# TuringLang/AdvancedVI.jl

Measured on AMD Instinct MI355X. Metric: ELBO-grad-estimates/sec, higher is better.
Workload: dtype f32

## Files before the change

### advancedvi.jl_amd/csrc/api_batch.hip

```cpp
#include "api_common.h"

bool graph_capturable(const mivi_ctx *c) {
  return c->target == TGT_DIAG_GAUSS || c->target == TGT_DENSE_GAUSS || c->target == TGT_FUNNEL || c->target == TGT_LOGREG;
}
mivi_status_t reserve_target(mivi_ctx *c, int M) {
  if (c->target == TGT_LOGREG && !logreg_reserve(c, M)) return fail(c, MIVI_ERR_HIP, "logistic regression: scratch allocation failed");
  return MIVI_OK;
}

static mivi_status_t record_chain(mivi_ctx *k, const void *params, uint64_t first, uint64_t stride, int cnt, const uint64_t *idx_ptr, void *value,
                                  void *grad) {
  Chain chn;
  chn.on = true;
  chn.estimates_only = true;
  mivi_status_t s = MIVI_OK;
  for (int i = 0; i < cnt && s == MIVI_OK; ++i) {
    RngArgs r = rng_of(k, first + (uint64_t)i * stride);
    if (idx_ptr) r.idx_ptr = idx_ptr;
    k->cur = i & 1;
    chn.has_next = (i + 1 < cnt);
    chn.next_rng = rng_of(k, first + ((uint64_t)i + 1) * stride);
    chn.next_rng.idx_ptr = r.idx_ptr;
    s = run_estimate(k, params, r, k->cfg.n_mc, 1, final_out(k, value, grad), &chn);
  }
// ... 205 lines not shown
    fs.stl = stl ? 1 : 0;
    if (st == steps - 1 && (value_last || grad_last)) { fs.lane_last = Llast - 1; fs.grad_last = grad_last; fs.value_last = value_last; }
    if (dist) { fs.parts = (char *)t.parts.p + (size_t)(overlap ? (st & 1) : 0) * (size_t)t.cap_LP * part_len * 4; fs.part_stride = (long long)part_len; }
    return fs;
  };
  ExchangePipe &pipe = c->fb_pipe;
  int handed = 0;
  auto step = [&](int st) -> mivi_status_t {
    const FbStep fs = make_step(st);
    if (overlap && (s = pipe.reuse(c, c->stream, st))) return s;
    fb_launch_eps(c, fs, st == 0, c->stream);
    fb_launch_compute(c, fs, c->stream);
    if (!dist) return MIVI_OK;
    hipStream_t xs = c->stream;
    if (overlap) {
      if ((s = pipe.hand_over(c, c->stream, st, &xs))) return s;
      handed = st + 1;
    }
    if ((s = dist_allreduce_f32(c, fs.parts, (size_t)fs.L * part_len, xs))) return s;
    fb_launch_finalize_parts(c, fs, xs);
    return overlap ? pipe.finish(c, st) : MIVI_OK;
  };
  s = MIVI_OK;
  for (int st = 0; st < steps && s == MIVI_OK; ++st) s = step(st);
  if (s) {
    pipe.join_after_error(c->stream, handed);
    return s;
  }
  if (overlap && (s = pipe.join(c, c->stream, steps))) return s;
  HIPCHK(c, hipGetLastError());
  return MIVI_OK;
}

mivi_status_t mivi::fb_objective(mivi_ctx *c, const void *params, uint64_t idx, int lanes, int entropy, void *values) {
  if (!fb_route(c, params, nullptr, nullptr) || c->M_total != c->cfg.n_mc) return MIVI_ERR_UNSUPPORTED;
  return fb_batch(c, params, idx, lanes, nullptr, nullptr, values, nullptr, entropy);
}

int32_t mivi_batch_lanes(const mivi_ctx_t *c, int32_t count) {
  if (!c || count <= 0) return 0;
  const int Lmax = switches().fb_lanes, steps = (count + Lmax - 1) / Lmax;
  return (count + steps - 1) / steps;
}

int32_t mivi_batch_info(const mivi_ctx_t *c, const void *params, int32_t what) {
  if (!c) return 0;
  if (what == 1) return 3;
  if (what == 2) return 4;
  if (what == 3) return c->exchange_lost ? 1 : 0;
  if (what == 4) return c->graph_records;
  if (what == 5) return live_allocations();
  if (what == 6) return live_handles();
  if (what == 7) return c->last_loop;
  return (what == 0 && params && fb_route(c, params, nullptr, nullptr)) ? 1 : 0;
}

mivi_status_t mivi_profile_batch(mivi_ctx_t *c, const void *params, int32_t lanes, int32_t reps, double *us_out) {
  if (!c || !params || lanes <= 0 || reps <= 0 || !us_out) return MIVI_ERR_BAD_ARG;
  if (mivi_status_t rs = refuse_non_gaussian(c, "mivi_profile_batch")) return rs;
  (void)hipSetDevice(c->cfg.device);
  if (!fb_route(c, params, nullptr, nullptr)) return fail(c, MIVI_ERR_UNSUPPORTED, "mivi_profile_batch: this configuration does not take the batch engine");
  if (lanes > switches().fb_lanes) lanes = switches().fb_lanes;
  char *o = (char *)c->tmp_out.p;
  mivi_status_t s = fb_batch(c, params, 1, lanes, o, o + 16, nullptr, nullptr);
  if (s) return s;
  const FbTab *tab = fb_prepare(c, c->cfg.n_mc, lanes);
  if (!tab) return fail(c, MIVI_ERR_HIP, "batch engine: work table allocation failed");
  FbStep fs{};
  fs.params = params; fs.M = c->cfg.n_mc; fs.L = lanes; fs.tab = tab;
  fs.rng = rng_of(c, 1);
  fs.grads = c->fb.grads.p; fs.grad_stride = (long long)mivi_params_len(c); fs.values = c->fb.values.p; fs.value_stride = 1; fs.lane_last = -1;
  fs.dense = c->target == TGT_DENSE_GAUSS ? 1 : 0;
  fs.stl = stl_entropy(c) ? 1 : 0;
  us_out[3] = us_out[4] = 0.0;
  EventTimer timer;
  for (int which = 0; which < 5; ++which) {
    if ((which == 3 && !fs.dense) || (which == 4 && !fs.stl)) continue;
    for (int r = -2; r < reps; ++r) {
      if (r == 0 && (s = timer.start(c, c->stream))) return s;
      if (which == 0) fb_launch_eps(c, fs, true, c->stream);
      else fb_launch_compute(c, fs, c->stream, which == 1 ? 1 : (which == 2 ? 2 : (which == 3 ? 4 : 8)));
    }
    double us = 0.0;
    if ((s = timer.stop_us(c, c->stream, &us))) return s;
    us_out[which] = us / reps;
  }
  HIPCHK(c, hipGetLastError());
  return MIVI_OK;
}

bool fb_dist_route(const mivi_ctx *c, const void *params, const void *grad) { return fb_route(c, params, grad, nullptr) && fb_whole_tiles(c, c->cfg.n_mc); }
mivi_status_t fb_batch_dist(mivi_ctx *c, const void *params, uint64_t idx0, int count, void *value, void *grad) {
  return fb_batch(c, params, idx0, count, value, grad, nullptr, nullptr, -1, true);
}

mivi_status_t mivi_estimate_gradient_each(mivi_ctx_t *c, const void *params, uint64_t idx0, int32_t count, void *values, void *grads) {
  if (!c || !params || !values || count <= 0) return MIVI_ERR_BAD_ARG;
  (void)hipSetDevice(c->cfg.device);
  if (c->target == TGT_NONE) return fail(c, MIVI_ERR_NO_TARGET, "no target set");
  if (fb_route(c, params, nullptr, grads)) return fb_batch(c, params, idx0, count, nullptr, nullptr, values, grads);
  const size_t plen = (size_t)mivi_params_len(c);
  mivi_status_t s = MIVI_OK;
  for (int i = 0; i < count && s == MIVI_OK; ++i)
    s = run_estimate(c, params, rng_of(c, idx0 + (uint64_t)i), c->cfg.n_mc, 1,
                     final_out(c, (char *)values + (size_t)i * c->esize, grads ? (void *)((char *)grads + (size_t)i * plen * c->esize) : c->tmp_out.p));
  return s;
// ... 128 lines not shown
```

### advancedvi.jl_amd/csrc/api_core.hip

```cpp
#include <atomic>
#include <climits>
#include <cstddef>
#include <cstdlib>

#include "api_common.h"

__global__ void k_acc_value_f32(double *acc, const float *v, double w, int first) { acc[0] = (first ? 0.0 : acc[0]) + w * (double)v[0]; }
__global__ void k_acc_value_f64(double *acc, const double *v, double w, int first) { acc[0] = (first ? 0.0 : acc[0]) + w * v[0]; }
__global__ void k_store_value_f32(float *out, const double *acc) { out[0] = (float)acc[0]; }
__global__ __launch_bounds__(256) void k_mean_values_f32(double *acc, const float *v, int n, double w) {
  __shared__ double part[256];
  double s = 0.0;
  for (int i = threadIdx.x; i < n; i += 256) s += (double)v[i];
  part[threadIdx.x] = s;
  __syncthreads();
  if (threadIdx.x == 0) {
    double t = 0.0;
    for (int i = 0; i < 256; ++i) t += part[i];
    acc[0] = w * t;
  }
}
__global__ void k_store_value_f64(double *out, const double *acc) { out[0] = acc[0]; }
__global__ void k_set_u64x2(uint64_t *dst, uint64_t a, uint64_t b, int n) { dst[0] = a; if (n > 1) dst[1] = b; }
__global__ void k_bump_u64(uint64_t *dst, uint64_t by) { dst[0] += by; }
__global__ void k_empty(int *sink) {
  extern __shared__ int lds_dyn[];
  if (sink && threadIdx.x == 0 && blockIdx.x == 0x7fffffff) sink[0] = lds_dyn[0];
}


mivi_status_t fail(mivi_ctx *c, mivi_status_t s, const char *msg) {
  if (c) c->err = msg;
  return s;
}

namespace mivi {
namespace {
enum SwitchKind {
  SW_PRESENCE,
  SW_ON_UNLESS_0,
  SW_OFF_UNLESS_1,
  SW_INT,
  SW_STRING
};
constexpr int kNoLo = INT_MIN, kNoHi = INT_MAX;
struct SwitchRow { const char *name; SwitchKind kind; size_t field; int def, lo, hi; const char *meaning; };
#define SW(f) offsetof(Switches, f)
const SwitchRow kSwitchTable[] = {
    {"MIVI_FR_GEN1", SW_PRESENCE, SW(fr_gen1), 0, 0, 0, "full-rank f32: first-generation tile kernels at every shape (lds_path_shape_ok)"},
    {"MIVI_STEIN_GEN1", SW_PRESENCE, SW(stein_gen1), 0, 0, 0, "Stein accumulation stage on the first-generation kernel (lds_stein_ok)"},
    {"MIVI_STL_GEN1", SW_PRESENCE, SW(stl_gen1), 0, 0, 0, "sticking-the-landing solve: not the second-generation packed solve (stl2_shape_ok)"},
    {"MIVI_STL_VALU", SW_PRESENCE, SW(stl_valu), 0, 0, 0, "first-generation solve on the vector ALU, not the 16-column look-ahead solve (launch_fr_stl)"},
    {"MIVI_LR_F32_LOGITS", SW_PRESENCE, SW(lr_f32_logits), 0, 0, 0, "logistic regression: f32-MFMA logits kernel (the one d % 4 != 0 takes), no operand planes"},
    {"MIVI_LR_NO_PLANES", SW_PRESENCE, SW(lr_no_planes), 0, 0, 0, "logistic regression: logits with X split in the tile (k_lr_logits_f16x2)"},
    {"MIVI_LR_NO_XPLANES", SW_PRESENCE, SW(lr_no_xplanes), 0, 0, 0, "logistic regression: X^T R with the splits made in the tile (k_lr_xtr_f16x2)"},
    {"MIVI_NO_FUSED_LOOP", SW_PRESENCE, SW(no_fused_loop), 0, 0, 0, "no launch-free loop kernels: batches and optimisation loops as graphs of launches"},
    {"MIVI_NO_FUSED_UPDATE", SW_PRESENCE, SW(no_fused_update), 0, 0, 0, "graph loop: the optimiser step as a kernel of its own, not in the VJP epilogue"},
    {"MIVI_FORCE_EXCHANGE_LOST", SW_PRESENCE, SW(force_exchange_lost), 0, 0, 0, "test hook (tests/test_gpu_loop_oracle.py): the first exchanging loop call counts as lost"},
    {"MIVI_BATCH_GEN3", SW_ON_UNLESS_0, SW(batch_gen3), 0, 0, 0, "=0: batches off the third-generation engine, on the lane-batched second-generation kernels"},
    {"MIVI_FB_STL", SW_ON_UNLESS_0, SW(fb_stl), 0, 0, 0, "=0: sticking-the-landing batches off the engine (lane-batched kernels + solves)"},
    {"MIVI_PROD_QUAD", SW_ON_UNLESS_0, SW(prod_quad), 0, 0, 0, "=0: four lanes' sampling products as k_fr_prod32m tiles, not k_fr_prod32q"},
    {"MIVI_P2P_DIRECT", SW_OFF_UNLESS_1, SW(p2p_direct), 0, 0, 0, "=1: sharded partials staged straight into the peers' buffers (mivi_p2p_partials_direct)"},
    {"MIVI_GRAPH_MIN", SW_INT, SW(graph_min), 6, kNoLo, kNoHi, "smallest full-rank batch that is captured as a graph (shorter: an eager chain)"},
    {"MIVI_CHAINS", SW_INT, SW(chains), 0, kNoLo, kNoHi, "> 0: that many interleaved contexts per batch (0: by shape)"},
    {"MIVI_FB_LANES", SW_INT, SW(fb_lanes), 80, 1, 256, "estimates per step of the batch engine"},
    {"MIVI_LANE_BATCH", SW_INT, SW(lane_batch), -1, kNoLo, kNoHi, "contexts per graph branch: 0 = every context on a branch of its own, 1 .. 4, < 0 = by shape"},
    {"MIVI_VJP_STRIP", SW_INT, SW(vjp_strip), 3, 0, 32, "tiles per workgroup of the lane-batched VJP (k_fr_vjp32s); 0 = one each (k_fr_vjp32m)"},
    {"MIVI_VJP_TILE", SW_INT, SW(vjp_tile), 0, kNoLo, kNoHi, "32 / 64 pins the second-generation VJP's tile size (0: by shape)"},
    {"MIVI_RCCL_LIB", SW_STRING, SW(rccl_lib), 0, 0, 0, "path of the RCCL library to load (unset: the loader's search)"},
#ifdef MIVI_DEV
    {"MIVI_FB_DBG", SW_PRESENCE, SW(fb_dbg), 0, 0, 0, "batch engine: per-workgroup clock stamps, summarised on stderr"},
    {"MIVI_STL_STAMPS", SW_PRESENCE, SW(stl_stamps), 0, 0, 0, "second-generation solve: per-block clock stamps on stderr"},
    {"MIVI_FB_KNOCK", SW_INT, SW(fb_knock), 0, kNoLo, kNoHi, "batch engine: work-skipping bits (operand loads / MFMAs / epilogue / stores)"},
    {"MIVI_FB_RING", SW_INT, SW(fb_ring), 0, kNoLo, kNoHi, "4 / 8 pins the engine product's ring depth (tools/fb_lane_curve.py)"},
    {"MIVI_KNOCK", SW_INT, SW(knock), 0, kNoLo, kNoHi, "second-generation kernels: work-skipping bits"},
#endif
};
#undef SW
Switches read_switches() {
  Switches s{};
  for (const SwitchRow &r : kSwitchTable) {
    const char *v = getenv(r.name);
    void *f = (char *)&s + r.field;
    switch (r.kind) {
      case SW_PRESENCE: *(bool *)f = v != nullptr; break;
      case SW_ON_UNLESS_0: *(bool *)f = !(v && atoi(v) == 0); break;
      case SW_OFF_UNLESS_1: *(bool *)f = v && atoi(v) == 1; break;
      case SW_INT: { const int x = v ? atoi(v) : r.def; *(int *)f = x < r.lo ? r.lo : (x > r.hi ? r.hi : x); break; }
      case SW_STRING: *(const char **)f = v; break;
    }
  }
  return s;
}
}
const Switches &switches() {
  static const Switches s = read_switches();
  return s;
}

bool grid_resident(const mivi_ctx *c, const void *kernel, int block, size_t dyn_lds, long long grid) {
  int nb = 0;
  if (hipOccupancyMaxActiveBlocksPerMultiprocessor(&nb, kernel, block, dyn_lds) != hipSuccess) { (void)hipGetLastError(); return false; }
  return c->n_cu > 0 && (long long)nb * c->n_cu >= grid;
}
}

static std::atomic<int32_t> g_live_allocations{0};
int32_t live_allocations() { return g_live_allocations.load(); }

void mivi::DevBuf::release() {
  if (owned && p) { (void)hipFree(p); --g_live_allocations; }
  p = nullptr; bytes = 0; owned = false;
}

mivi_status_t ensure(mivi_ctx *c, DevBuf &b, size_t bytes, bool zero, bool fine_grained) {
  if (b.bytes >= bytes && b.p) return MIVI_OK;
  b.release();
  if (bytes == 0) bytes = 16;
  void *p = nullptr;
  HIPCHK(c, fine_grained ? hipExtMallocWithFlags(&p, bytes, hipDeviceMallocFinegrained) : hipMalloc(&p, bytes));
  ++g_live_allocations;
  b.p = p; b.bytes = bytes; b.owned = true;
  if (zero) HIPCHK(c, hipMemsetAsync(b.p, 0, bytes, c->stream));
  return MIVI_OK;
}

mivi_status_t ensure_zeroed(mivi_ctx *c, DevBuf &b, size_t bytes) {
// ... 527 lines not shown
```

### advancedvi.jl_amd/csrc/fr_planes.h

```cpp
#pragma once
#include "device_common.h"

namespace mivi {

typedef float f32x16 __attribute__((ext_vector_type(16)));
typedef float f32x4 __attribute__((ext_vector_type(4)));
typedef _Float16 f16x8 __attribute__((ext_vector_type(8)));
typedef _Float16 f16x2 __attribute__((ext_vector_type(2)));
typedef unsigned u32x4v __attribute__((ext_vector_type(4)));

constexpr int kFrag = 512;
constexpr int kSplitProducts = 3;
constexpr float kEpsScale = 2048.f;
constexpr float kEpsInv = 1.f / 2048.f;

#define FB_GLDS16(gptr, lptr, off)                                                                         \
  __builtin_amdgcn_global_load_lds((const __attribute__((address_space(1))) void *)(gptr),                 \
                                   (__attribute__((address_space(3))) void *)(lptr), 16, off, 0)

template <int N>
__device__ __forceinline__ void fb_wait_vm() {
  __builtin_amdgcn_s_waitcnt((N & 15) | (7 << 4) | (15 << 8) | ((N >> 4) << 14));
  asm volatile("" ::: "memory");
}
// ... 30 lines not shown
  return (float)hh[odd] + (float)ll[odd];
}
__device__ __forceinline__ void fb_store_frag(unsigned *dst, const float *x) {
  u32x4v uh, ul;
  fb_split2(x, uh, ul);
  store16_wt(dst, uh);
  store16_wt(dst + 256, ul);
}

constexpr int kStageW = 16 * 256;

template <int WJ>
struct FbFrags {
  u32x4v A[2][2], B[WJ][2];
};
__device__ __forceinline__ f32x16 fb_mma(const u32x4v &a, const u32x4v &b, const f32x16 &c) {
  return __builtin_amdgcn_mfma_f32_32x32x16_f16(__builtin_bit_cast(f16x8, a), __builtin_bit_cast(f16x8, b), c, 0, 0, 0);
}
template <int WJ>
__device__ __forceinline__ void fb_group(const FbFrags<WJ> &F, f32x16 (&acc)[2][WJ]) {
  constexpr int PA[3] = {1, 0, 0}, PB[3] = {0, 1, 0};
#pragma unroll
  for (int p = 0; p < 3; ++p)
#pragma unroll
    for (int i = 0; i < 2; ++i)
#pragma unroll
      for (int j = 0; j < WJ; ++j) acc[i][j] = fb_mma(F.A[i][PA[p]], F.B[j][PB[p]], acc[i][j]);
}

template <int OFF>
__device__ __forceinline__ void fb_group_read_asm(f32x16 &acc0, f32x16 &acc1, const FbFrags<1> &Fc, FbFrags<1> &Fn, unsigned ab, unsigned bb) {
  static_assert(OFF >= 0 && OFF + 3072 < 65536, "ds_read_b128 offset field");
  asm volatile(
      "v_mfma_f32_32x32x16_f16 %[c0], %[a0l], %[bh], %[c0]\n\t"
      "ds_read_b128 %[n0h], %[ab] offset:%[o0]\n\t"
      "ds_read_b128 %[n0l], %[ab] offset:%[o1]\n\t"
      "v_mfma_f32_32x32x16_f16 %[c1], %[a1l], %[bh], %[c1]\n\t"
      "ds_read_b128 %[n1h], %[ab] offset:%[o2]\n\t"
      "ds_read_b128 %[n1l], %[ab] offset:%[o3]\n\t"
      "v_mfma_f32_32x32x16_f16 %[c0], %[a0h], %[bl], %[c0]\n\t"
      "ds_read_b128 %[nbh], %[bb] offset:%[o0]\n\t"
      "v_mfma_f32_32x32x16_f16 %[c1], %[a1h], %[bl], %[c1]\n\t"
      "ds_read_b128 %[nbl], %[bb] offset:%[o1]\n\t"
      "v_mfma_f32_32x32x16_f16 %[c0], %[a0h], %[bh], %[c0]\n\t"
      "v_mfma_f32_32x32x16_f16 %[c1], %[a1h], %[bh], %[c1]\n\t"
      "s_waitcnt lgkmcnt(0)"
      : [c0] "+v"(acc0), [c1] "+v"(acc1), [n0h] "=&v"(Fn.A[0][0]), [n0l] "=&v"(Fn.A[0][1]), [n1h] "=&v"(Fn.A[1][0]), [n1l] "=&v"(Fn.A[1][1]),
        [nbh] "=&v"(Fn.B[0][0]), [nbl] "=&v"(Fn.B[0][1])
      : [a0h] "v"(Fc.A[0][0]), [a0l] "v"(Fc.A[0][1]), [a1h] "v"(Fc.A[1][0]), [a1l] "v"(Fc.A[1][1]), [bh] "v"(Fc.B[0][0]), [bl] "v"(Fc.B[0][1]),
        [ab] "v"(ab), [bb] "v"(bb), [o0] "n"(OFF), [o1] "n"(OFF + 1024), [o2] "n"(OFF + 2048), [o3] "n"(OFF + 3072)
      : "memory");
}

template <int WJ>
__device__ __forceinline__ void fb_read_frags(const unsigned *lds, int slot, int wm, int wn, int lane, FbFrags<WJ> &F) {
  const unsigned *cur = lds + slot * kStageW + 4 * lane;
#pragma unroll
  for (int i = 0; i < 2; ++i)
#pragma unroll
    for (int p = 0; p < 2; ++p) F.A[i][p] = *(const u32x4v *)(cur + ((2 * wm + i) * 2 + p) * 256);
#pragma unroll
  for (int j = 0; j < WJ; ++j)
#pragma unroll
    for (int p = 0; p < 2; ++p) F.B[j][p] = *(const u32x4v *)(cur + (8 + (WJ * wn + j) * 2 + p) * 256);
}

}
```

### advancedvi.jl_amd/csrc/kernels_fullrank_batch.hip

```cpp
#include <algorithm>
#include <cstdlib>
#include <type_traits>
#include <cstdio>
#include <vector>

#include "device_common.h"
#include "fr_elem.h"
#include "fr_planes.h"

#ifndef FB_VK
#define FB_VK 0
#endif
#ifndef FB_WJ
#define FB_WJ 1
#endif

namespace mivi {

struct FbArgs {
  int d, M, L;
  int dT, MT;
  const float *params;
  const float *t_mean, *t_istd;
  unsigned *CA;
// ... 542 lines not shown
#pragma unroll
        for (int g2 = 0; g2 < 2; ++g2) {
          float x[8];
#pragma unroll
          for (int e = 0; e < 8; ++e) x[e] = I[(16 * g2 + 8 * (e >> 2) + 4 * h + (e & 3)) * LDC + l31] * s;
          fb_store_frag(WVl + ((size_t)r32[i] * nmg + 2 * cb32 + g2) * kFrag + 4 * lane, x);
        }
      }
    }
  }
  FB_STAMP(a, 3);
  if (!kDG && !kSU && (flags & 1) && wn == 0 && lane < 32) {
    const int nrb = d >> 5;
#pragma unroll
    for (int i = 0; i < 2; ++i) {
      const int r = 32 * r32[i] + lane;
      float lg, bad;
      logdet_block32(r < a.dT ? a.params[a.dT + (size_t)r * a.dT + r] : 1.f, lg, bad);
      if (lane == 0) {
        a.ld_part[r32[i]] = (double)lg;
        a.ld_part[nrb + r32[i]] = (double)bad;
      }
    }
  }
}

__device__ __forceinline__ void fb_value_block(const FbArgs &a, int l, double *red) {
  const int d = a.d;
  ValueIn vin{};
  vin.ell_const = a.ell_const;
  vin.ell_part = a.ell_part + (size_t)l * a.ell_stride;
  vin.n_ell_part = (d >> 5) * (a.M >> 5);
  vin.he_part = a.he_part + (size_t)l * a.he_stride;
  vin.n_he_part = (d >> 6) * (a.M >> 5);
  vin.ld_part = a.ld_part;
  vin.n_ld_part = d >> 5;
  OutArgs out{};
  const bool last = l == a.lane_last && a.value_last;
  out.value = last ? a.value_last : a.values + (size_t)l * a.value_stride;
  if (a.parts) {
    out.partials_mode = 1;
    out.partials = a.parts + (size_t)l * a.part_stride;
    out.scalars_off = (int64_t)d + (int64_t)(d >> 7) * ((d >> 7) + 1) / 2 * 16384;
  }
  out.ent_kind = a.ent_kind;
  out.M_total = a.M_total;
  out.M_local = a.MT;
  out.status = a.status;
  const float *pp = a.params;
  const int dT = a.dT;
  finalize_value_block<float, 256, false>(dT, vin, out, (int64_t)dT + (int64_t)dT * dT, [pp, dT](int i) { return pp[dT + (size_t)i * dT + i]; }, red);
}

template <int WJ, int NRV, int TABW, int WPE, bool PART = false>
__global__ __launch_bounds__(512 / WJ, WPE / WJ) void k_fb_vjp(FbArgs a) {
  static_assert(WJ == 1, "the transposing B reads are written for the 64 x 32 wave tiles");
  constexpr int LDC = 36, NF = WJ, kPW = 2 * WJ;
  constexpr int NR = NRV;
  constexpr int kBody = (NR * kStageW > 16 * kImgW / 2) ? NR * kStageW : 16 * kImgW / 2;
  __shared__ __attribute__((aligned(16))) unsigned lds[kBody + TABW];
  float *wf = reinterpret_cast<float *>(lds + kBody);
  const int tid = threadIdx.x, lane = tid & 63, l31 = lane & 31, h = lane >> 5;
  const int w = __builtin_amdgcn_readfirstlane(tid >> 6);
  const int wm = w / (4 / WJ), wn = w % (4 / WJ);
  if ((int)blockIdx.x < a.L) {
    if (tid < 256) fb_value_block(a, (int)blockIdx.x, reinterpret_cast<double *>(lds));
    return;
  }
  const __attribute__((address_space(4))) int *wp = (const __attribute__((address_space(4))) int *)a.work + 4 * ((int)blockIdx.x - a.L);
  const int ln = wp[0], rc = wp[1];
  const int rb = rc & 0xffff, cb = rc >> 16;
  const int d = a.d, M = a.M, nmg = M >> 4, dT = a.dT;
  const int row0 = rb * 128, col0 = cb * 128;
  const bool last = ln == a.lane_last && a.grad_last;
  float *grad = last ? a.grad_last : a.grads + (size_t)ln * a.grad_stride;
  const bool upper = a.write_upper || last;
  const int G = nmg;
  const int NB = M >> 7;
  const unsigned *sp[NF];
  unsigned btr;
  {
    const int G4 = lane >> 4, c16 = lane & 15;
    const int kgpar = G4 & 1, hq = G4 >> 1, hp = c16 & 1, half = (c16 >> 1) & 1, sl = 4 * hq + (c16 >> 2);
    btr = 16u * (unsigned)(8 * (2 * hp + kgpar) + ((sl & 7) ^ (4 * hp))) + 8u * (unsigned)half;
  }
#pragma unroll
  for (int f = 0; f < NF; ++f) {
    const int fs = NF * w + f, fr = fs & 3;
    if (fs < 4) {
      sp[f] = a.WV + (size_t)ln * a.plane_stride + ((size_t)((row0 >> 5) + fr) * nmg) * kFrag + 4 * lane;
    } else {
      const int m8 = lane >> 3, s8 = m8 >> 2, hp = (m8 >> 1) & 1, kgpar = m8 & 1, sl = 8 * s8 + ((lane & 7) ^ (4 * hp));
      sp[f] = a.epsP + (size_t)ln * a.plane_stride + ((size_t)((col0 >> 4) + 2 * fr + kgpar)) * kFrag + 4 * (sl + 32 * hp);
    }
  }
  int gi = 0;
  const int bstep_odd = (d >> 4) * kFrag - 64;
  constexpr int kMaxNBv = 16;
  float twi[kMaxNBv];
  auto load_table = [&]() {
    if (tid < 128) {
      const float *wi = a.winv + (size_t)ln * (size_t)NB * d + row0 + tid;
#pragma unroll
      for (int r = 0; r < kMaxNBv; ++r) twi[r] = wi[(size_t)(r < NB ? r : NB - 1) * d];
    }
    asm volatile("" ::: "memory");
  };
  auto build_table = [&]() {
    if (tid < 128) {
// ... 44 lines not shown
  int cj[WJ];
#pragma unroll
  for (int j = 0; j < WJ; ++j) cj[j] = (col0 >> 5) + WJ * wn + j;
  const bool work = cj[0] <= ri[1];
  bool dg[2];
#pragma unroll
  for (int i = 0; i < 2; ++i) {
    dg[i] = false;
#pragma unroll
    for (int j = 0; j < WJ; ++j) dg[i] = dg[i] || ri[i] == cj[j];
  }
  f32x16 acc[2][WJ];
#pragma unroll
  for (int i = 0; i < 2; ++i)
#pragma unroll
    for (int j = 0; j < WJ; ++j)
#pragma unroll
      for (int r = 0; r < 16; ++r) acc[i][j][r] = 0.f;
  double rsd[2] = {0.0, 0.0};
  float rcur[2] = {0.f, 0.f};
  auto after_group = [&](auto S, int g, const FbFrags<WJ> &F) {
    if (__builtin_expect(dg[0] || dg[1], 0)) {
#pragma unroll
      for (int i = 0; i < 2; ++i)
        if (dg[i]) {
#pragma unroll
          for (int e = 0; e < 8; ++e) rcur[i] += fb_unsplit2(F.A[i][0], F.A[i][1], e);
        }
    }
    if constexpr (decltype(S)::value == 3 || decltype(S)::value == -1) {
      if (((g + 1) & 7) == 0 && g + 1 < G) {
        const float *wr = wf + ((g >> 3) << 7) + 64 * wm;
#pragma unroll
        for (int i = 0; i < 2; ++i) {
#pragma unroll
          for (int q = 0; q < 4; ++q) {
            const f32x4 f4 = *(const f32x4 *)(wr + 32 * i + 8 * q + 4 * h);
#pragma unroll
            for (int j = 0; j < WJ; ++j)
#pragma unroll
              for (int c = 0; c < 4; ++c) acc[i][j][4 * q + c] *= f4[c];
          }
          rsd[i] = (rsd[i] + (double)rcur[i]) * (double)wr[32 * i + l31];
          rcur[i] = 0.f;
        }
        asm volatile("" ::: "memory");
      }
    }
  };
  auto compute = [&](auto S, int g, const FbFrags<WJ> &F) {
    if (!(FB_VK & 32)) fb_group<WJ>(F, acc);
    after_group(S, g, F);
  };
  {
    FB_STAMP(a, 0);
    FB_NOTE(a, 4, G);
    load_table();
#pragma unroll
    for (int s0 = 0; s0 < NR - 1; ++s0) issue(s0);
    fb_wait_vm<kPW * (NR - 1)>();
    build_table();
    int slot = 0;
    for (int g = 0; g < G; ++g) {
      if (g == 1) FB_STAMP(a, 1);
      if (g + NR - 2 < G) fb_wait_vm<kPW * (NR - 2)>();
      else if (NR > 3 && g + 1 < G) fb_wait_vm<kPW>();
      else fb_wait_vm<0>();
      fb_barrier();
      if (g + NR - 1 < G) issue(slot == 0 ? NR - 1 : slot - 1);
      if (work) {
        FbFrags<WJ> F;
        read_frags(slot, F);
        compute(std::integral_constant<int, -1>{}, g, F);
      }
      slot = slot == NR - 1 ? 0 : slot + 1;
    }
  }
  fb_barrier();
  FB_STAMP(a, 2);
  if ((FB_VK & 128)) return;
  float *Cs = reinterpret_cast<float *>(lds) + w * kImgW;
  const float *wfin = wf + (NB - 1) * 128 + 64 * wm;
  const double invM = 1.0 / (double)a.M_total;
  const bool pow2M = (a.M_total & (a.M_total - 1)) == 0;
  const float invMe = (float)invM * kEpsInv;
  const double direct = direct_entropy_coeff(a.ent_kind);
  const int i4 = 4 * (lane & 7);
#pragma unroll
  for (int i = 0; i < 2; ++i) {
#pragma unroll
    for (int j = 0; j < WJ; ++j) {
      if (cj[j] > ri[i] || 32 * ri[i] >= dT) continue;
      const bool diag = ri[i] == cj[j];
      const int rbase = 32 * ri[i], cbase = 32 * cj[j];
#pragma unroll
      for (int q = 0; q < 4; ++q) {
        const f32x4 v = {acc[i][j][4 * q], acc[i][j][4 * q + 1], acc[i][j][4 * q + 2], acc[i][j][4 * q + 3]};
        *(f32x4 *)(Cs + l31 * LDC + 8 * q + 4 * h) = v;
      }
      const f32x4 ff = *(const f32x4 *)(wfin + 32 * i + i4);
#pragma unroll
      for (int p = 0; p < 4; ++p) {
        const int n = 8 * p + (lane >> 3);
        const int gi = rbase + i4, gj = cbase + n;
        float cjj = 1.f;
        if (diag && gj >= gi && gj < gi + 4) cjj = a.params[dT + (size_t)gj * dT + gj];
        const f32x4 v = *(const f32x4 *)(Cs + n * LDC + i4) * ff;
// ... 230 lines not shown
  const int d = fb_pad(c->cfg.d), M = fb_pad(s.M), L = s.L;
  FbArgs a = fb_args(c, s.params, s.M);
  a.L = L;
  a.rng = s.rng;
  a.obj = s.obj;
  const int gx = (d / 64) * (M / 32) / 2;
  a.n_riders = with_cplanes ? (4 * (d / 32) + gx - 1) / gx : 0;
  hipLaunchKernelGGL(k_fb_eps, dim3(gx, L + a.n_riders), dim3(512), 0, stream, a);
}
void fb_launch_pplanes(mivi_ctx *c, hipStream_t stream) {
  FbArgs a = fb_args(c, nullptr, c->cfg.n_mc);
  hipLaunchKernelGGL(k_fb_pplanes, dim3(c->cfg.d / 32, 4), dim3(512), 0, stream, a);
}
void fb_launch_tplanes(mivi_ctx *c, hipStream_t stream) {
  FbArgs a = fb_args(c, nullptr, c->cfg.n_mc);
  hipLaunchKernelGGL(k_fb_tplanes, dim3(c->cfg.d / 32, 4), dim3(512), 0, stream, a);
}
void fb_launch_compute(mivi_ctx *c, const FbStep &s, hipStream_t stream, int which) {
  const FbTab &tb = *s.tab;
  FbArgs a = fb_args(c, s.params, s.M);
  a.L = s.L;
  a.grads = (float *)s.grads; a.grad_stride = s.grad_stride;
  a.values = (float *)s.values; a.value_stride = s.value_stride;
  a.grad_last = (float *)s.grad_last; a.value_last = (float *)s.value_last; a.lane_last = s.lane_last;
  a.write_upper = s.write_upper;
  a.parts = (float *)s.parts; a.part_stride = s.part_stride;
  if (s.obj) { a.ent_kind = s.ent_kind; a.M_total = s.M; }
#ifdef MIVI_DEV
  static long long *dbg_buf = nullptr;
  const bool dbg_on = switches().fb_dbg;
  if (dbg_on && !dbg_buf) (void)hipMalloc(&dbg_buf, 2 * 8192 * 8 * sizeof(long long));
  auto dump = [&](const char *name, int n) {
    if (!dbg_on) return;
    (void)hipStreamSynchronize(stream);
    std::vector<long long> h((size_t)n * 8);
    (void)hipMemcpy(h.data(), dbg_buf, h.size() * 8, hipMemcpyDeviceToHost);
    long long t0 = h[0], t3 = 0;
    for (int i = 0; i < n; ++i) { t0 = std::min(t0, h[(size_t)i * 8]); t3 = std::max(t3, h[(size_t)i * 8 + 3]); }
    double pro = 0, loop = 0, epi = 0, pg = 0; long long gs = 0;
    for (int i = 0; i < n; ++i) { const long long *r = &h[(size_t)i * 8]; pro += r[1] - r[0]; loop += r[2] - r[1]; epi += r[3] - r[2]; gs += r[4]; }
    pg = loop / (double)gs;
    fprintf(stderr, "[fbdbg] %s: %d workgroups, span %.2f us | mean prologue %.2f us, main loop %.2f us (%.3f us per group), epilogue %.2f us | last start %.2f us\n", name, n, (t3 - t0) * 0.01, pro / n * 0.01, loop / n * 0.01, pg * 0.01, epi / n * 0.01, 0.0);
    std::vector<long long> st; for (int i = 0; i < n; ++i) st.push_back(h[(size_t)i * 8] - t0);
    std::sort(st.begin(), st.end());
    fprintf(stderr, "[fbdbg]   starts (us): p25 %.2f p50 %.2f p75 %.2f p90 %.2f max %.2f\n", st[n / 4] * 0.01, st[n / 2] * 0.01, st[3 * n / 4] * 0.01, st[9 * n / 10] * 0.01, st[n - 1] * 0.01);
  };
  a.dbg = dbg_on ? dbg_buf : nullptr;
  a.knock = switches().fb_knock;
#endif
  a.work = (const int4 *)tb.prod.p; a.n_work = tb.n_prod;
  const int n_cu = c->n_cu > 0 ? c->n_cu : 256;
  auto own_cu_for = [&](int n, bool equal_tiles) {
#ifdef MIVI_DEV
    if (switches().fb_ring == 4) return false;
    if (switches().fb_ring == 8) return true;
#endif
    const int gmax = fb_pad(c->cfg.d) / 16;
    const int thr10 = gmax <= 32 ? 10 : (gmax <= 64 ? 10 + (gmax - 32) * 7 / 32 : kOwnCuTilesPerCU10 + (gmax - 64 < 64 ? gmax - 64 : 64) * 5 / 64);
    return !equal_tiles && n > n_cu && 10 * (long long)n <= (long long)thr10 * n_cu;
  };
  auto prod = [&](auto MODE, int n) {
    constexpr int md = decltype(MODE)::value;
    if (own_cu_for(n, md == FB_DENSE_G)) hipLaunchKernelGGL((k_fb_prod<kWJ, md, 8>), dim3(n), dim3(512 / kWJ), 0, stream, a);
    else hipLaunchKernelGGL((k_fb_prod<kWJ, md, 4>), dim3(n), dim3(512 / kWJ), 0, stream, a);
  };
  if (s.dense) {
    if (which & 1) prod(std::integral_constant<int, FB_DENSE_R>{}, tb.n_prod);
    a.work = (const int4 *)tb.prod2.p; a.n_work = tb.n_prod2;
    if (which & 4) prod(std::integral_constant<int, FB_DENSE_G>{}, tb.n_prod2);
  } else if (which & 1) {
    prod(std::integral_constant<int, FB_DIAG>{}, tb.n_prod);
#ifdef MIVI_DEV
    dump("k_fb_prod<DIAG>", tb.n_prod);
#endif
  }
  if (s.stl && (which & 8)) {
    a.work = (const int4 *)tb.prod3.p; a.n_work = tb.n_prod;
    prod(std::integral_constant<int, FB_STL_U>{}, tb.n_prod);
  }
  a.work = (const int4 *)tb.vjp.p; a.n_work = tb.n_vjp;
  if (s.values_only) {
    if (which & 2) hipLaunchKernelGGL((k_fb_vjp<kWJ, 3, 256, 6>), dim3(s.L), dim3(512 / kWJ), 0, stream, a);
    return;
  }
  if (which & 2) {
    if (s.parts) {
      if (a.M <= 256) hipLaunchKernelGGL((k_fb_vjp<kWJ, 3, 256, 6, true>), dim3(tb.n_vjp + s.L), dim3(512 / kWJ), 0, stream, a);
      else hipLaunchKernelGGL((k_fb_vjp<kWJ, 3, 2048, 4, true>), dim3(tb.n_vjp + s.L), dim3(512 / kWJ), 0, stream, a);
    }
    else if (a.M <= 256) hipLaunchKernelGGL((k_fb_vjp<kWJ, 3, 256, 6>), dim3(tb.n_vjp + s.L), dim3(512 / kWJ), 0, stream, a);
    else hipLaunchKernelGGL((k_fb_vjp<kWJ, 3, 2048, 4>), dim3(tb.n_vjp + s.L), dim3(512 / kWJ), 0, stream, a);
#ifdef MIVI_DEV
    dump("k_fb_vjp", tb.n_vjp);
#endif
  }
}

void fb_launch_finalize_parts(mivi_ctx *c, const FbStep &s, hipStream_t stream) {
  FbArgs a = fb_args(c, s.params, s.M);
  a.L = s.L;
  a.grads = (float *)s.grads; a.grad_stride = s.grad_stride;
  a.values = (float *)s.values; a.value_stride = s.value_stride;
  a.grad_last = (float *)s.grad_last; a.value_last = (float *)s.value_last; a.lane_last = s.lane_last;
  a.write_upper = s.write_upper;
  a.parts = (float *)s.parts; a.part_stride = s.part_stride;
  hipLaunchKernelGGL(k_fb_finalize_parts, dim3(c->cfg.d + 1, s.L), dim3(256), 0, stream, a);
}

}
```

### advancedvi.jl_amd/csrc/mivi_internal.h

```cpp
#pragma once
#include <hip/hip_runtime.h>
#include <math.h>
#include <stdint.h>

#include <string>
#include <utility>
#include <vector>

#include "../../include/mivi.h"
#include "philox.h"
#include "switches.h"

namespace mivi {

constexpr double kLog2Pi = 1.8378770664093454835606594728112;

struct RngArgs {
  uint64_t seed;
  uint64_t idx_base;
  const uint64_t *idx_ptr;
  int m_offset;
};

enum TargetKind : int {
// ... 395 lines not shown
  std::vector<char> h_Z, h_G, h_ell;

  int cap_M = 0;
  mivi::DevBuf eps[2], epsT[2], ell_part[2], he_part[2], sc_part[2], ld_part[2];
  mivi::DevBuf tabA, tabB, tabD;
  mivi::DevBuf stl_CT, stl_Dinv;
  mivi::DevBuf stl_F;
  bool want_stl_pack = false, stl_pack_done = false;
  mivi::DevBuf stl_X;
  mivi::DevBuf lds_tabV, lds_tabV64, lds_tabS;
  int lds_nV = 0, lds_nV64 = 0, lds_nS = 0, lds_M = -1;
  bool d_idx_valid = false;
  uint64_t d_idx_expect = 0;
  mivi::DevBuf lds_tabSt;
  int lds_nSt = 0, lds_st_d = -1;
  mivi::ValueJob *defer_value = nullptr;
  bool value_deferred = false;
  int he_n[2] = {0, 0};
  int nA = 0, nB = 0, nD = 0, tab_M = -1;
  int cur = 0;
  int mf_nblk = 0;
  mivi::DevBuf Z, W, RT, ell, X;
  mivi::DevBuf row_part, status, d_idx, acc, tmp_params, tmp_out;
  mivi::DevBuf obj_vals;
  mivi::DevBuf stein_A, stein_g;
  mivi::DevBuf sg_S, sg_d;
  int sg_cap = 0;
  mivi::DevBuf ms_work, ms_part;
  mivi::DevBuf bam_host;
  mivi::DevBuf ngd_est, natgrad_host;
  mivi::DevBuf h2_acc;
  mivi::DevBuf lowr_E, lowr_V, lowr_prep, lowr_sx, lowr_part;
  int base = MIVI_BASE_NORMAL;
  double base_nu = 0.0, base_c0 = 0.0, base_H = 0.0;
  mivi::DevBuf bd_U, bd_R;
  mivi::DevBuf lp_dinv, lp_scal, lp_work, lp_host;
  mivi::DevBuf dog_part;
  const uint64_t *idx_src = nullptr;
  mivi::EpsSpec pre;
  long long *dbg = nullptr;
  int dP = 0, MP = 0;

  mivi::GraphCache graph;
  int graph_records = 0;
  mivi::FbTables fb;

  int idx_stride = 1;
  bool is_child = false;
  int n_cu = 0;
  size_t lds_max = 64 * 1024;
  bool exchange_lost = false;
  int last_status_bits = 0;
  int last_loop = 0;
  mivi::DevBuf snap;
  mivi_ctx *kids[kMaxKids] = {};
  int n_kids = 0;
  unsigned long long target_gen = 0, kid_gen = ~0ull;
  bool dist_capture_refused = false;
  bool dist_direct = false;
  bool dist_lane4 = false;
  mivi::LaneRecorder *rec = nullptr;
  int lane_id = 0;
  mivi::DevBuf kid_out[kMaxKids];

  ~mivi_ctx() { (void)mivi_comm_destroy(this); graph.drop(); }
};

#pragma GCC visibility push(hidden)
mivi_status_t ensure(mivi_ctx *c, mivi::DevBuf &b, size_t bytes, bool zero, bool fine_grained = false);
mivi_status_t ensure_zeroed(mivi_ctx *c, mivi::DevBuf &b, size_t bytes);
mivi_status_t upload(mivi_ctx *c, mivi::DevBuf &b, const void *src, size_t bytes);
int32_t live_allocations();
mivi_status_t make_stream(mivi_ctx *c, mivi::Stream &s, bool own_queue);
mivi_status_t make_event(mivi_ctx *c, mivi::Event &e, bool timing);
mivi_status_t ensure_pipe(mivi_ctx *c, mivi::ExchangePipe &p, bool own_queue);
int32_t live_handles();
#pragma GCC visibility pop

template <typename F>
inline auto by_dtype(const mivi_ctx *c, F &&f) { return c->cfg.dtype == MIVI_F32 ? f(float{}) : f(double{}); }

namespace mivi {

struct ValueJob;
void launch_mf_main(mivi_ctx *c, const void *params, const RngArgs &rng, int M, int want_grad, const void *G,
                    const ValueIn &vin, const OutArgs &out, const ValueJob *prev = nullptr);
enum DeviceLoopId : int { LOOP_GRAPH = 0, LOOP_MF_SGD = 1, LOOP_LR_SMALL = 2, LOOP_MF_GEN = 3, LOOP_FR_SMALL = 4, LOOP_FR_ROWS = 5, LOOP_MF_FUNNEL_SGD = 6,
                          LOOP_MANY = 16 };
struct LoopBufs {
  void *value, *grad;
  double *rec, *area;
};
struct ManyRun {
  uint64_t seed, idx0;
  double eta, ell_const;
};
struct ManyLaunch {
  int n_runs;
  const ManyRun *runs;
  int *status;
  const void *t_mean, *t_istd;
  const uint8_t *y;
  const void *X;
  long long x_stride;
};
constexpr int kManyGridY = 65535;
// ... 193 lines not shown
```

Baseline: 352,900.

## Add software-pipelined VJP loop overlapping LDS fragment reads with MFMAs

Adds a pipelined variant of the batch-engine VJP kernel. A hand-scheduled inline-asm group interleaves the MFMAs of the current k-group with the ds_read and transposing ds_read_b64_tr_b16 loads of the next group's fragments, using a four-slot ring and double-buffered fragments. The launch picks this variant when M > 256 or the tile count is at most twice the CU count, and it uses 4 waves per EU instead of 6 for the small-M case. The aim is to hide LDS latency behind matrix work, at the cost of more registers and ring LDS, lower occupancy, and a fragile hand-written asm schedule.

```diff
diff --git a/advancedvi.jl_amd/csrc/api_batch.hip b/advancedvi.jl_amd/csrc/api_batch.hip
--- a/advancedvi.jl_amd/csrc/api_batch.hip
+++ b/advancedvi.jl_amd/csrc/api_batch.hip
@@ -281,6 +281,7 @@
   if (what == 5) return live_allocations();
   if (what == 6) return live_handles();
   if (what == 7) return c->last_loop;
+  if (what == 8) return c->last_vjp_pipelined;
   return (what == 0 && params && fb_route(c, params, nullptr, nullptr)) ? 1 : 0;
 }
 
diff --git a/advancedvi.jl_amd/csrc/api_core.hip b/advancedvi.jl_amd/csrc/api_core.hip
--- a/advancedvi.jl_amd/csrc/api_core.hip
+++ b/advancedvi.jl_amd/csrc/api_core.hip
@@ -72,7 +72,7 @@
     {"MIVI_FB_DBG", SW_PRESENCE, SW(fb_dbg), 0, 0, 0, "batch engine: per-workgroup clock stamps, summarised on stderr"},
     {"MIVI_STL_STAMPS", SW_PRESENCE, SW(stl_stamps), 0, 0, 0, "second-generation solve: per-block clock stamps on stderr"},
     {"MIVI_FB_KNOCK", SW_INT, SW(fb_knock), 0, kNoLo, kNoHi, "batch engine: work-skipping bits (operand loads / MFMAs / epilogue / stores)"},
-    {"MIVI_FB_RING", SW_INT, SW(fb_ring), 0, kNoLo, kNoHi, "4 / 8 pins the engine product's ring depth (tools/fb_lane_curve.py)"},
+    {"MIVI_FB_RING", SW_INT, SW(fb_ring), 0, kNoLo, kNoHi, "units 4 / 8 pin the engine product's ring depth (tools/fb_lane_curve.py), tens 3 / 4 the VJP's plain / pipelined loop (tools/fb_vjp_loops.py)"},
     {"MIVI_KNOCK", SW_INT, SW(knock), 0, kNoLo, kNoHi, "second-generation kernels: work-skipping bits"},
 #endif
 };
diff --git a/advancedvi.jl_amd/csrc/fr_planes.h b/advancedvi.jl_amd/csrc/fr_planes.h
--- a/advancedvi.jl_amd/csrc/fr_planes.h
+++ b/advancedvi.jl_amd/csrc/fr_planes.h
@@ -106,6 +106,36 @@
       : "memory");
 }
 
+template <int OFF>
+__device__ __forceinline__ void fb_group_read_tr_asm(f32x16 &acc0, f32x16 &acc1, const FbFrags<1> &Fc, FbFrags<1> &Fn, unsigned ab, unsigned bt) {
+  static_assert(OFF >= 0 && OFF + 3072 < 65536, "ds_read offset field");
+  uint2 bh0, bh1, bl0, bl1;
+  asm volatile(
+      "v_mfma_f32_32x32x16_f16 %[c0], %[a0l], %[bh], %[c0]\n\t"
+      "ds_read_b128 %[n0h], %[ab] offset:%[o0]\n\t"
+      "ds_read_b128 %[n0l], %[ab] offset:%[o1]\n\t"
+      "v_mfma_f32_32x32x16_f16 %[c1], %[a1l], %[bh], %[c1]\n\t"
+      "ds_read_b128 %[n1h], %[ab] offset:%[o2]\n\t"
+      "ds_read_b128 %[n1l], %[ab] offset:%[o3]\n\t"
+      "v_mfma_f32_32x32x16_f16 %[c0], %[a0h], %[bl], %[c0]\n\t"
+      "ds_read_b64_tr_b16 %[bh0], %[bt] offset:%[o0]\n\t"
+      "ds_read_b64_tr_b16 %[bh1], %[bt] offset:%[t1]\n\t"
+      "v_mfma_f32_32x32x16_f16 %[c1], %[a1h], %[bl], %[c1]\n\t"
+      "ds_read_b64_tr_b16 %[bl0], %[bt] offset:%[o1]\n\t"
+      "ds_read_b64_tr_b16 %[bl1], %[bt] offset:%[t3]\n\t"
+      "v_mfma_f32_32x32x16_f16 %[c0], %[a0h], %[bh], %[c0]\n\t"
+      "v_mfma_f32_32x32x16_f16 %[c1], %[a1h], %[bh], %[c1]\n\t"
+      "s_waitcnt lgkmcnt(0)"
+      : [c0] "+v"(acc0), [c1] "+v"(acc1), [n0h] "=&v"(Fn.A[0][0]), [n0l] "=&v"(Fn.A[0][1]), [n1h] "=&v"(Fn.A[1][0]), [n1l] "=&v"(Fn.A[1][1]),
+        [bh0] "=&v"(bh0), [bh1] "=&v"(bh1), [bl0] "=&v"(bl0), [bl1] "=&v"(bl1)
+      : [a0h] "v"(Fc.A[0][0]), [a0l] "v"(Fc.A[0][1]), [a1h] "v"(Fc.A[1][0]), [a1l] "v"(Fc.A[1][1]), [bh] "v"(Fc.B[0][0]), [bl] "v"(Fc.B[0][1]),
+        [ab] "v"(ab), [bt] "v"(bt), [o0] "n"(OFF), [o1] "n"(OFF + 1024), [o2] "n"(OFF + 2048), [o3] "n"(OFF + 3072), [t1] "n"(OFF + 512),
+        [t3] "n"(OFF + 1536)
+      : "memory");
+  Fn.B[0][0] = u32x4v{bh0.x, bh0.y, bh1.x, bh1.y};
+  Fn.B[0][1] = u32x4v{bl0.x, bl0.y, bl1.x, bl1.y};
+}
+
 template <int WJ>
 __device__ __forceinline__ void fb_read_frags(const unsigned *lds, int slot, int wm, int wn, int lane, FbFrags<WJ> &F) {
   const unsigned *cur = lds + slot * kStageW + 4 * lane;
diff --git a/advancedvi.jl_amd/csrc/kernels_fullrank_batch.hip b/advancedvi.jl_amd/csrc/kernels_fullrank_batch.hip
--- a/advancedvi.jl_amd/csrc/kernels_fullrank_batch.hip
+++ b/advancedvi.jl_amd/csrc/kernels_fullrank_batch.hip
@@ -618,9 +618,10 @@
   finalize_value_block<float, 256, false>(dT, vin, out, (int64_t)dT + (int64_t)dT * dT, [pp, dT](int i) { return pp[dT + (size_t)i * dT + i]; }, red);
 }
 
-template <int WJ, int NRV, int TABW, int WPE, bool PART = false>
+template <int WJ, int NRV, int TABW, int WPE, bool PART = false, bool PIPE = false>
 __global__ __launch_bounds__(512 / WJ, WPE / WJ) void k_fb_vjp(FbArgs a) {
   static_assert(WJ == 1, "the transposing B reads are written for the 64 x 32 wave tiles");
+  static_assert(!PIPE || NRV == 4, "the pipelined loop is unrolled by its four-slot ring");
   constexpr int LDC = 36, NF = WJ, kPW = 2 * WJ;
   constexpr int NR = NRV;
   constexpr int kBody = (NR * kStageW > 16 * kImgW / 2) ? NR * kStageW : 16 * kImgW / 2;
@@ -771,7 +772,48 @@
     if (!(FB_VK & 32)) fb_group<WJ>(F, acc);
     after_group(S, g, F);
   };
-  {
+  if constexpr (PIPE) {
+    const unsigned lds0 = (unsigned)(uintptr_t)lds;
+    const unsigned ab0 = lds0 + 16u * lane + (2 * wm) * 2 * 1024, bt0 = lds0 + (8 + 2 * wn) * 1024 + btr;
+    auto step = [&](auto S, auto VM, auto ISS, int g, const FbFrags<WJ> &Fc, FbFrags<WJ> &Fn) {
+      constexpr int sl = decltype(S)::value;
+      fb_wait_vm<kPW * decltype(VM)::value>();
+      fb_barrier();
+      if constexpr (decltype(ISS)::value) issue(sl);
+      if (work) {
+        fb_group_read_tr_asm<((sl + 1) & 3) * kStageW * 4>(acc[0][0], acc[1][0], Fc, Fn, ab0, bt0);
+        if constexpr (sl == 3) {
+          if (((g + 1) & 7) == 0) asm volatile("s_nop 15\n\ts_nop 7" : "+v"(acc[0][0]), "+v"(acc[1][0])::"memory");
+        }
+        after_group(S, g, Fc);
+      }
+    };
+    FB_STAMP(a, 0);
+    FB_NOTE(a, 4, G);
+    load_table();
+    static_for<0, 4>([&](auto S) { issue(decltype(S)::value); });
+    fb_wait_vm<kPW * 4>();
+    build_table();
+    fb_wait_vm<kPW * 3>();
+    fb_barrier();
+    FB_STAMP(a, 1);
+    FbFrags<WJ> F0, F1;
+    if (work) read_frags(0, F0);
+    int g = 0;
+    for (; g + 4 < G; g += 4) {
+      static_for<0, 4>([&](auto S) {
+        constexpr int sv = decltype(S)::value;
+        if constexpr (sv % 2 == 0) step(S, std::integral_constant<int, 2>{}, FbT{}, g + sv, F0, F1);
+        else step(S, std::integral_constant<int, 2>{}, FbT{}, g + sv, F1, F0);
+      });
+    }
+    static_for<0, 3>([&](auto S) {
+      constexpr int sv = decltype(S)::value;
+      if constexpr (sv % 2 == 0) step(S, std::integral_constant<int, 2 - sv>{}, FbN{}, g + sv, F0, F1);
+      else step(S, std::integral_constant<int, 2 - sv>{}, FbN{}, g + sv, F1, F0);
+    });
+    if (work) compute(std::integral_constant<int, 3>{}, g + 3, F1);
+  } else {
     FB_STAMP(a, 0);
     FB_NOTE(a, 4, G);
     load_table();
@@ -1108,12 +1150,20 @@
   const int n_cu = c->n_cu > 0 ? c->n_cu : 256;
   auto own_cu_for = [&](int n, bool equal_tiles) {
 #ifdef MIVI_DEV
-    if (switches().fb_ring == 4) return false;
-    if (switches().fb_ring == 8) return true;
+    if (switches().fb_ring % 10 == 4) return false;
+    if (switches().fb_ring % 10 == 8) return true;
 #endif
     const int gmax = fb_pad(c->cfg.d) / 16;
     const int thr10 = gmax <= 32 ? 10 : (gmax <= 64 ? 10 + (gmax - 32) * 7 / 32 : kOwnCuTilesPerCU10 + (gmax - 64 < 64 ? gmax - 64 : 64) * 5 / 64);
     return !equal_tiles && n > n_cu && 10 * (long long)n <= (long long)thr10 * n_cu;
+  };
+  auto vjp_pipelined_for = [&](int n_tiles, int M, int d) {
+#ifdef MIVI_DEV
+    if (switches().fb_ring / 10 == 3) return false;
+    if (switches().fb_ring / 10 == 4) return true;
+#endif
+    (void)d;
+    return M > 256 || n_tiles <= 2 * n_cu;
   };
   auto prod = [&](auto MODE, int n) {
     constexpr int md = decltype(MODE)::value;
@@ -1137,15 +1187,24 @@
   a.work = (const int4 *)tb.vjp.p; a.n_work = tb.n_vjp;
   if (s.values_only) {
     if (which & 2) hipLaunchKernelGGL((k_fb_vjp<kWJ, 3, 256, 6>), dim3(s.L), dim3(512 / kWJ), 0, stream, a);
+    c->last_vjp_pipelined = 0;
     return;
   }
   if (which & 2) {
-    if (s.parts) {
-      if (a.M <= 256) hipLaunchKernelGGL((k_fb_vjp<kWJ, 3, 256, 6, true>), dim3(tb.n_vjp + s.L), dim3(512 / kWJ), 0, stream, a);
-      else hipLaunchKernelGGL((k_fb_vjp<kWJ, 3, 2048, 4, true>), dim3(tb.n_vjp + s.L), dim3(512 / kWJ), 0, stream, a);
-    }
-    else if (a.M <= 256) hipLaunchKernelGGL((k_fb_vjp<kWJ, 3, 256, 6>), dim3(tb.n_vjp + s.L), dim3(512 / kWJ), 0, stream, a);
-    else hipLaunchKernelGGL((k_fb_vjp<kWJ, 3, 2048, 4>), dim3(tb.n_vjp + s.L), dim3(512 / kWJ), 0, stream, a);
+    const bool pipe = vjp_pipelined_for(tb.n_vjp, a.M, a.d);
+    c->last_vjp_pipelined = pipe ? 1 : 0;
+    auto vjp = [&](auto PARTS) {
+      constexpr bool pt = decltype(PARTS)::value;
+      const dim3 grid(tb.n_vjp + s.L), block(512 / kWJ);
+      if (pipe) {
+        if (a.M <= 256) hipLaunchKernelGGL((k_fb_vjp<kWJ, 4, 256, 4, pt, true>), grid, block, 0, stream, a);
+        else hipLaunchKernelGGL((k_fb_vjp<kWJ, 4, 2048, 4, pt, true>), grid, block, 0, stream, a);
+      }
+      else if (a.M <= 256) hipLaunchKernelGGL((k_fb_vjp<kWJ, 3, 256, 6, pt>), grid, block, 0, stream, a);
+      else hipLaunchKernelGGL((k_fb_vjp<kWJ, 3, 2048, 4, pt>), grid, block, 0, stream, a);
+    };
+    if (s.parts) vjp(FbT{});
+    else vjp(FbN{});
 #ifdef MIVI_DEV
     dump("k_fb_vjp", tb.n_vjp);
 #endif
diff --git a/advancedvi.jl_amd/csrc/mivi_internal.h b/advancedvi.jl_amd/csrc/mivi_internal.h
--- a/advancedvi.jl_amd/csrc/mivi_internal.h
+++ b/advancedvi.jl_amd/csrc/mivi_internal.h
@@ -471,6 +471,7 @@
   bool exchange_lost = false;
   int last_status_bits = 0;
   int last_loop = 0;
+  int last_vjp_pipelined = 0;
   mivi::DevBuf snap;
   mivi_ctx *kids[kMaxKids] = {};
   int n_kids = 0;
```

Result: no change. 353,900 (median of 2 runs) (+0.3%).
